# wenzhang-dev/bitcaskDB

Hardware: AMD Instinct MI355X
Metric: WAL record decode+CRC GiB/s (device-resident), 4 KiB values, 1/2/4/8 MI355X (higher is better)
Workload: dtype u8; 1 GPU; config B: 1073743514 B WAL segment per GPU, NsSize 20, 100 B keys, 4 KiB values, device-resident decode+CRC+record parse; seg_bytes=1073743514, records=253846, fragments=286402, parallelism=one independent segment per GPU x1

## Files before the change

### bitcaskdb_amd/csrc/bcw_decode.hip

```cpp
#include <hip/hip_runtime.h>

#include <cstdint>

#include "bcw_internal.h"
#include "bcw_parse.h"

namespace bcw {

enum { M_FIRST_BAD = 0,
       M_NE = 1,
       M_NFRAGS = 4, M_DONE_CRC = 5,
       M_T_CRC0 = 10, M_T_FIN = 11,
       M_ABORT = 12,
       M_BAD_CRC = 14,
       M_BAD_TYPE = 15 };

__device__ __forceinline__ uint32_t rotl32(uint32_t x, int r) { return (x << r) | (x >> (32 - r)); }

__device__ __forceinline__ void read_header(const uint8_t* __restrict__ seg, uint64_t seg_len, uint64_t off,
                                            uint32_t& crc, uint32_t& len, uint32_t& type) {
  const uint64_t a = off & ~3ull;
  uint32_t w0, w1, w2;
  if (a + 12 <= seg_len) {
    const uint32_t* q = reinterpret_cast<const uint32_t*>(seg + a);
    w0 = q[0]; w1 = q[1]; w2 = q[2];
  } else {
    uint32_t b[12];
#pragma unroll
    for (int i = 0; i < 12; ++i) b[i] = (a + i < seg_len) ? seg[a + i] : 0u;
    w0 = b[0] | b[1] << 8 | b[2] << 16 | b[3] << 24;
    w1 = b[4] | b[5] << 8 | b[6] << 16 | b[7] << 24;
    w2 = b[8] | b[9] << 8 | b[10] << 16 | b[11] << 24;
  }
  const uint32_t sh = (uint32_t)(off & 3);
  crc = __builtin_amdgcn_alignbyte(w1, w0, sh);
  const uint32_t t = __builtin_amdgcn_alignbyte(w2, w1, sh);
  len = t & 0xffffu;
  type = (t >> 16) & 0xffu;
}

// ... 408 lines not shown
}
__device__ __forceinline__ uint32_t apply_fwd(const uint32_t* __restrict__ fwd, uint32_t lane, uint32_t x) {
  const uint8_t* b = reinterpret_cast<const uint8_t*>(fwd);
  const uint32_t lane4 = 4u * lane;
  auto at = [&](int i) -> uint32_t {
    const uint32_t sh = 4 * i >= 8 ? (x >> (4 * i - 8)) : (x << (8 - 4 * i));
    return *reinterpret_cast<const uint32_t*>(b + (((sh & 0xf00u) | lane4) + 4096u * (uint32_t)i));
  };
  const uint32_t r0 = at(0), r1 = at(1), r2 = at(2), r3 = at(3), r4 = at(4), r5 = at(5), r6 = at(6), r7 = at(7);
  return xor3(xor3(r0, r1, r2), xor3(r3, r4, r5), r6) ^ r7;
}
__device__ __forceinline__ uint32_t apply_op(const uint32_t* __restrict__ c, uint32_t x) {
  uint32_t r = 0;
#pragma unroll
  for (int i = 0; i < 8; ++i) r ^= c[i * 16 + ((x >> (4 * i)) & 15u)];
  return r;
}

__device__ __forceinline__ uint4 load16_slow(const uint8_t* __restrict__ seg, uint64_t seg_len, int64_t o) {
  uint64_t lo = 0, hi = 0;
#pragma unroll 1
  for (int i = 0; i < 16; ++i) {
    const int64_t q = o + i;
    const uint64_t byte = (q >= 0 && (uint64_t)q < seg_len) ? seg[q] : 0u;
    if (i < 8) lo |= byte << (8 * i); else hi |= byte << (8 * (i - 8));
  }
  return make_uint4((uint32_t)lo, (uint32_t)(lo >> 32), (uint32_t)hi, (uint32_t)(hi >> 32));
}
__device__ __forceinline__ uint4 load16_safe(const uint8_t* __restrict__ seg, uint64_t seg_len, int64_t o) {
  if (o >= 0 && (uint64_t)o + 16 <= seg_len) return *reinterpret_cast<const uint4*>(seg + o);
  return load16_slow(seg, seg_len, o);
}


template <int N>
__device__ __forceinline__ uint32_t reg_byte(const uint32_t (&h)[N], uint32_t pos) {
  uint32_t t[N];
#pragma unroll
  for (int i = 0; i < N; ++i) t[i] = h[i];
  const uint32_t wi = pos >> 2;
  int n = N;
#pragma unroll
  for (int bit = 0; bit < 6; ++bit) {
    if (n <= 1) break;
    const bool hi = (wi >> bit) & 1u;
#pragma unroll
    for (int i = 0; i < (N + 1) / 2; ++i) {
      if (i < (n + 1) / 2) t[i] = (2 * i + 1 < n) ? (hi ? t[2 * i + 1] : t[2 * i]) : t[2 * i];
    }
    n = (n + 1) / 2;
  }
  return (t[0] >> (8u * (pos & 3u))) & 0xffu;
}

constexpr int kHeadWords = 16;
constexpr int kTailWords = 8;

__device__ __attribute__((noinline)) uint32_t walk_byte(const uint8_t* __restrict__ seg, const Frag* __restrict__ frags,
                                                        uint32_t start_off, uint32_t f_first, uint32_t f_last,
                                                        uint64_t pos) {
  uint64_t beg = 0;
  for (uint32_t cf = f_first;; ++cf) {
    const Frag f = frags[cf];
    if (pos < beg + f.len || cf >= f_last)
      return seg[(uint64_t)start_off + (uint64_t)f.blk * kBlock + f.start + (pos - beg)];
    beg += f.len;
  }
}

struct RegReader {
  uint32_t h[kHeadWords];
  uint32_t t[kTailWords];
  uint32_t nhead;
  uint64_t tstart;
  uint64_t tend;
  const uint8_t* seg;
  const Frag* frags;
  uint32_t start_off;
  uint32_t f_first, f_last;
  __device__ __forceinline__ uint32_t operator()(uint64_t pos) {
    if (pos < nhead) return reg_byte(h, (uint32_t)pos);
    if (pos >= tstart && pos < tend) return reg_byte(t, (uint32_t)(pos - tstart));
    return walk_byte(seg, frags, start_off, f_first, f_last, pos);
  }
};

template <int N>
__device__ __forceinline__ void load_words(const uint8_t* __restrict__ seg, uint64_t seg_len, uint64_t base,
                                           uint32_t (&w)[N]) {
  if (base + 4u * N <= seg_len) {
#pragma unroll
    for (int k = 0; k < N / 4; ++k) {
      uint4 v;
      __builtin_memcpy(&v, seg + base + 16 * k, 16);
      w[4 * k + 0] = v.x; w[4 * k + 1] = v.y; w[4 * k + 2] = v.z; w[4 * k + 3] = v.w;
    }
  } else {
#pragma unroll
    for (int k = 0; k < N / 4; ++k) {
      const uint4 v = load16_safe(seg, seg_len, (int64_t)(base + 16 * k));
      w[4 * k + 0] = v.x; w[4 * k + 1] = v.y; w[4 * k + 2] = v.z; w[4 * k + 3] = v.w;
    }
  }
}

struct EmitArgs {
  const uint8_t* seg;
  uint64_t seg_len;
  bcw_decode_params p;
  const Frag* frags;
  const uint32_t* fbase;
  const uint32_t* rbase;
  const uint2* bsum;
  bcw_record_table tab;
  uint64_t* misc;
  uint32_t kb_flags;
  uint64_t* kb_stamps;
};


struct EmitState {
  uint64_t acc;
  int64_t nzb;
  uint32_t nzk, nzs;
  uint64_t rec;
};
__device__ __forceinline__ uint2 emit_prefetch(const EmitArgs& A, uint64_t b0, uint32_t lane) {
  return b0 > lane ? A.bsum[b0 - 1 - lane] : make_uint2(0xffff0000u, kSumHasE);
}

__device__ __forceinline__ EmitState emit_state(const EmitArgs& A, uint64_t b0, uint32_t lane, uint2 s, uint32_t rec) {
  EmitState st{0, -1, 0, 0, rec};
  uint64_t acc = 0;
  for (uint64_t top = b0; top > 0;) {
    if (top != b0) {
      const uint64_t q = top - 1 - lane;
      s = top > lane ? A.bsum[q] : make_uint2(0xffff0000u, kSumHasE);
    }
    const uint64_t he = __ballot((s.y & kSumHasE) != 0u);
    const uint32_t stop = he ? (uint32_t)__builtin_ctzll(he) : 63u;
    const bool contrib = lane <= stop;
    uint32_t ta = contrib ? (s.x & 0xffffu) : 0u;
#pragma unroll
    for (int d = 32; d >= 1; d >>= 1) ta += (uint32_t)__shfl_xor((int)ta, d, 64);
    acc += (uint32_t)__builtin_amdgcn_readfirstlane(ta);
    const uint64_t nzm = __ballot(contrib && (s.x >> 16) != 0xffffu);
    if (nzm) {
      const uint32_t L = 63u - __builtin_clzll(nzm);
      st.nzb = (int64_t)(top - 1 - L);
      st.nzk = (uint32_t)__builtin_amdgcn_readlane((int)(s.x >> 16), L);
      st.nzs = (uint32_t)__builtin_amdgcn_readlane((int)(s.y & 0xffffu), L);
    }
    if (he) break;
    top = top > 64 ? top - 64 : 0;
  }
  st.acc = acc;
  return st;
}

template <bool NOSTORE = false, bool NOPARSE = false, typename Hook>
__device__ __forceinline__ void emit_chunks(const EmitArgs& A, const EmitState& es, uint64_t f0, uint64_t f1,
                                            uint32_t lane, Hook&& hook) {
  if (f0 >= f1) {
    hook();
    return;
  }
  const Frag* __restrict__ frags = A.frags;
  const uint32_t start_off = A.p.start_off;
  uint64_t acc = es.acc, off = 0;
  uint32_t first = 0;
  if (es.nzb >= 0) {
    off = (uint64_t)start_off + (uint64_t)es.nzb * kBlock + es.nzs;
    first = A.fbase[es.nzb] + es.nzk;
  }
  uint64_t rec = es.rec;
  const bool hint = A.p.mode == BCW_MODE_HINT;
  for (uint64_t c0 = f0; c0 < f1; c0 += 64) {
    const uint64_t g = c0 + lane;
    const bool valid = g < f1;
    const uint4 fr = reinterpret_cast<const uint4*>(frags)[valid ? g : f1 - 1];
    if (c0 == f0) hook();
    Frag f;
    __builtin_memcpy(&f, &fr, sizeof f);
    if (!valid) f = Frag{};
    const uint32_t len = valid ? f.len : 0u;
    const uint64_t D = (uint64_t)start_off + (uint64_t)f.blk * kBlock + f.start;
    const bool isE = valid && (f.type == BCW_RECORD_FULL || f.type == BCW_RECORD_LAST);
    const uint64_t E = __ballot(isE);
    const uint64_t NZ = __ballot(valid && len > 0);
    const uint32_t S = wave_add_scan(len, lane);
    const uint64_t below = (lane == 0) ? 0ull : (~0ull >> (64 - lane));
    const uint64_t pm = E & below;
    const int prev = pm ? 63 - __builtin_clzll(pm) : -1;
    const uint32_t S_prev = __shfl(S, prev < 0 ? 0 : prev, 64);
    const uint64_t between = (uint64_t)(S - len) - (prev < 0 ? 0u : S_prev);
    const uint64_t acc_before = (prev < 0 ? acc : 0ull) + between;
    const uint64_t range = prev < 0 ? below : (below & ~(~0ull >> (63 - prev)));
    const uint64_t nzr = NZ & range;
    const int fnz = nzr ? __builtin_ctzll(nzr) : 0;
    const uint64_t D_fnz = __shfl(D, fnz, 64);
    const uint64_t V = __ballot(valid);
    const int last_valid = V ? 63 - __builtin_clzll(V) : -1;
    const uint32_t S_tot = __shfl(S, last_valid < 0 ? 0 : last_valid, 64);
// ... 17 lines not shown
      }
    }
    uint64_t foff;
    uint32_t ffrag;
    if (acc_before == 0) { foff = D; ffrag = (uint32_t)g; }
    else if (prev < 0 && acc > 0) { foff = off; ffrag = first; }
    else { foff = D_fnz; ffrag = (uint32_t)(c0 + fnz); }
    const bool full = f.type == BCW_RECORD_FULL;
    const uint32_t src = full ? (uint32_t)g : ffrag;
    const bool src_here = src >= c0 && src < c0 + 64;
    const uint32_t sw0 = (uint32_t)__shfl((int)f.blk, src_here ? (int)(src - c0) : (int)lane, 64);
    const uint32_t sw1 = (uint32_t)__shfl((int)((uint32_t)f.start | ((uint32_t)f.len << 16)),
                                          src_here ? (int)(src - c0) : (int)lane, 64);
    const bool nx_here = src + 1u >= c0 && src + 1u < c0 + 64;
    const uint32_t sx0 = (uint32_t)__shfl((int)f.blk, nx_here ? (int)(src + 1u - c0) : (int)lane, 64);
    const uint32_t sx1 = (uint32_t)__shfl((int)((uint32_t)f.start | ((uint32_t)f.len << 16)),
                                          nx_here ? (int)(src + 1u - c0) : (int)lane, 64);
    if (isE) {
      const uint64_t size = full ? (uint64_t)len : acc_before + len;
      const uint64_t r = rec + __builtin_popcountll(E & below);
      Frag fs = f;
      if (!full) {
        if (src_here) { fs.blk = sw0; fs.start = (uint16_t)sw1; fs.len = (uint16_t)(sw1 >> 16); }
        else fs = frags[src];
      }
      RegReader rd;
      const uint64_t a0 = (uint64_t)start_off + (uint64_t)fs.blk * kBlock + fs.start;
      uint64_t want = size < 64u ? size : 64u;
      if (want > fs.len) want = fs.len;
      rd.nhead = (uint32_t)want;
      load_words(A.seg, A.seg_len, a0, rd.h);
      rd.tstart = rd.tend = ~0ull;
      if (hint) {
        uint64_t nt = size < 32u ? size : 32u;
        if (nt > len) nt = len;
        rd.tstart = size - nt;
        load_words(A.seg, A.seg_len, D + len - nt, rd.t);
      } else if (want < (size < 64u ? size : 64u)) {
        Frag f2;
        if (nx_here) { f2.blk = sx0; f2.start = (uint16_t)sx1; f2.len = (uint16_t)(sx1 >> 16); }
        else f2 = frags[src + 1u];
        load_words(A.seg, A.seg_len, (uint64_t)start_off + (uint64_t)f2.blk * kBlock + f2.start, rd.t);
        uint64_t n2 = f2.len < 32u ? f2.len : 32u;
        if (n2 > size - want) n2 = size - want;
        rd.tstart = want;
        rd.tend = want + n2;
      } else {
#pragma unroll
        for (int k = 0; k < kTailWords; ++k) rd.t[k] = 0;
      }
      rd.seg = A.seg; rd.frags = frags; rd.start_off = start_off;
      rd.f_first = src; rd.f_last = (uint32_t)g;
      uint8_t status, hdr, flags, etag_off;
      uint64_t key_len, val_len, meta_len, expire, aux0, aux1;
      if (NOPARSE) {
        status = 0; hdr = (uint8_t)rd.h[0]; flags = (uint8_t)rd.h[5]; etag_off = 0;
        key_len = rd.h[6] ^ rd.h[9]; val_len = rd.h[7] ^ rd.h[12]; meta_len = rd.h[8] ^ rd.h[15]; expire = rd.h[10];
        aux0 = rd.t[0]; aux1 = rd.t[1];
      } else {
        parse_record(A.p, rd, size, status, hdr, flags, etag_off, key_len, val_len, meta_len, expire, aux0, aux1);
      }
      const bcw_record_table& tab = A.tab;
      if (NOSTORE) {
        if (status == 0xeeu) tab.foff[r] = foff ^ size ^ expire ^ aux0 ^ aux1 ^ key_len ^ val_len ^ meta_len ^ hdr ^ flags ^ etag_off;
      } else if (r < tab.capacity) {
        tab.foff[r] = foff;
        tab.size[r] = size;
        tab.expire[r] = expire;
        if (tab.aux0) tab.aux0[r] = aux0;
        if (tab.aux1) tab.aux1[r] = aux1;
        tab.key_len[r] = (uint32_t)key_len;
        tab.val_len[r] = (uint32_t)val_len;
        tab.meta_len[r] = (uint32_t)meta_len;
        tab.first_frag[r] = src;
        tab.emit_frag[r] = (uint32_t)g;
        tab.hdr_size[r] = hdr;
        tab.flags[r] = flags;
        tab.etag_off[r] = etag_off;
        tab.status[r] = status;
      }
      if (status != BCW_ST_OK) atomicMin((unsigned long long*)&A.misc[M_FIRST_BAD], (unsigned long long)r);
    }
    rec += __builtin_popcountll(E);
    acc = acc2;
    off = off2;
    first = first2;
  }
}

struct ItemMeta {
  uint64_t bb;
  uint2 s;
  uint32_t f0, f1, rec;
};
__device__ __forceinline__ uint32_t ld_const(const uint32_t* p, uint64_t i) {
  return ((const __attribute__((address_space(4))) uint32_t*)p)[i];
}
__device__ __forceinline__ ItemMeta item_meta(const EmitArgs& A, uint64_t it, uint64_t bpw, uint64_t cb0, uint64_t cb1,
                                              uint32_t lane) {
  ItemMeta m;
  m.bb = cb0 + it * bpw < cb1 ? cb0 + it * bpw : cb1 - 1;
  const uint64_t be = m.bb + bpw < cb1 ? m.bb + bpw : cb1;
  m.s = emit_prefetch(A, m.bb, lane);
  m.f0 = ld_const(A.fbase, m.bb);
  m.f1 = ld_const(A.fbase, be);
  m.rec = ld_const(A.rbase, m.bb);
  return m;
}

__device__ __forceinline__ void finalize(const EmitArgs& A, uint64_t nblocks, uint64_t frag_cap, uint32_t tail_panic, uint64_t gen,
                         bcw_decode_result* __restrict__ res, uint32_t lane) {
  uint64_t* misc = A.misc;
  const uint64_t bad_crc = __hip_atomic_load(&misc[M_BAD_CRC], __ATOMIC_RELAXED, __HIP_MEMORY_SCOPE_AGENT);
  const uint64_t bad_type = __hip_atomic_load(&misc[M_BAD_TYPE], __ATOMIC_RELAXED, __HIP_MEMORY_SCOPE_AGENT);
  const uint64_t fb = __hip_atomic_load(&misc[M_FIRST_BAD], __ATOMIC_RELAXED, __HIP_MEMORY_SCOPE_AGENT);
  const uint64_t nfr = __hip_atomic_load(&misc[M_NFRAGS], __ATOMIC_RELAXED, __HIP_MEMORY_SCOPE_AGENT);
  const uint64_t abort_site = __hip_atomic_load(&misc[M_ABORT], __ATOMIC_RELAXED, __HIP_MEMORY_SCOPE_AGENT);
  const uint64_t err = bad_crc < bad_type ? bad_crc : bad_type;
  uint64_t lim = err < frag_cap ? err : frag_cap;
  uint64_t nrec = __hip_atomic_load(&misc[M_NE], __ATOMIC_RELAXED, __HIP_MEMORY_SCOPE_AGENT);
  if (lim < nfr && abort_site == 0ull) {
    uint64_t lo = 0, hi = nblocks;
    while (hi - lo > 1) {
      const uint64_t step = (hi - lo + 63) / 64;
      const uint64_t q = lo + (uint64_t)lane * step;
      const bool le = q < hi && A.fbase[q] <= lim;
      const uint64_t m = __ballot(le);
      const uint32_t L = m ? 63u - __builtin_clzll(m) : 0u;
      lo = lo + (uint64_t)L * step;
      hi = lo + step < hi ? lo + step : hi;
    }
    uint64_t cnt = 0;
    for (uint64_t c0 = A.fbase[lo]; c0 < lim; c0 += 64) {
      const uint64_t g = c0 + lane;
      const uint32_t ty = g < lim ? A.frags[g].type : 0u;
      cnt += (uint64_t)__builtin_popcountll(__ballot(ty == BCW_RECORD_FULL || ty == BCW_RECORD_LAST));
    }
    nrec = (uint64_t)A.rbase[lo] + cnt;
  }
  if (lane != 0) return;
  bcw_decode_result r{};
  r.n_records = nrec;
  r.n_records_total = nrec;
  r.err_frag = err;
  r.err_class = err == ~0ull ? BCW_ERR_NONE : (bad_crc <= bad_type ? BCW_ERR_CRC : BCW_ERR_TYPE);
  r.n_frags = err != ~0ull ? err + 1 : nfr;
  if (r.err_class == BCW_ERR_NONE && tail_panic) r.err_class = BCW_ERR_PANIC;
  if (abort_site != 0ull) {
    r.err_class = BCW_ERR_INTERNAL;
    r.err_frag = abort_site;
    r.n_records = r.n_records_total = 0;
    nrec = 0;
  }
  r.err_file_off = 0;
  if (err != ~0ull && err < frag_cap && abort_site == 0ull) {
    const Frag f = A.frags[err];
    r.err_file_off = (uint64_t)A.p.start_off + (uint64_t)f.blk * kBlock + f.start - kHdr;
  }
  r.first_bad_record = fb < nrec ? (int32_t)(fb < 0x7fffffffull ? fb : 0x7fffffffull) : -1;
  r.n_blocks = nblocks;
  r.retry_frag_capacity = (nfr > frag_cap && abort_site == 0ull) ? nfr : 0;
  r.generation = gen;
  *res = r;
  if (abort_site != 0ull) misc[M_NFRAGS] = 0;
  misc[M_DONE_CRC] = 0;
  misc[M_BAD_CRC] = ~0ull;
  misc[M_FIRST_BAD] = ~0ull;
  misc[M_BAD_TYPE] = ~0ull;
  misc[M_ABORT] = 0;
}

struct StreamFrag {
  int64_t gs, ge;
  uint32_t J;
};

struct SliceLane2 {
  uint32_t base;
  uint32_t sel[4];
};
__device__ __forceinline__ SliceLane2 slice_lane2(uint32_t lane) {
  SliceLane2 s;
  const uint32_t g = (lane >> 3) & 3u, copy = lane & 7u;
  s.base = 0;
#pragma unroll
  for (uint32_t k = 0; k < 4; ++k) {
    const uint32_t slot = (k + g) & 3u;
    s.base |= (slot * 32u + copy * 4u) << (8u * k);
    s.sel[k] = 0x0c0c0000u | ((4u + slot) << 8) | k;
  }
  return s;
}
// ... 240 lines not shown
      const float d = fminf(fmaxf(rintf((wy - 65536.0f) / 256.0f), -51.0f), 64.0f);
      xb->w[y] = (uint32_t)(65536 + 256 * (int32_t)d);
    }
    xb->t[y] = 0;
    xb->n[y] = 0;
  }
}

template <int ABL = 0>
__global__ __launch_bounds__(kCrcThreads) void k_crc(const uint8_t* __restrict__ seg, uint64_t seg_len,
                                                     uint32_t start_off, uint64_t nblocks,
                                                     const uint32_t* __restrict__ fbase, uint8_t* __restrict__ fok,
                                                     const uint4* __restrict__ srec,
                                                     uint64_t frag_cap, Tables tabs, EmitArgs ea,
                                                     uint32_t tail_panic, uint64_t gen,
                                                     bcw_decode_result* __restrict__ res,
                                                     uint64_t* __restrict__ misc, uint64_t cb0, uint64_t cb1,
                                                     uint32_t nwg_total, const uint32_t* __restrict__ wstart,
                                                     XBal* __restrict__ xb) {
  __shared__ __attribute__((aligned(16))) uint32_t lds[kS2Image];
  __shared__ CrcTail s_tail;
  __shared__ uint32_t s_wdone;
  __shared__ uint32_t s_eq;
  __shared__ __attribute__((aligned(16))) uint32_t s_rem[kCrcWaves];
  __shared__ uint32_t s_sdone;
  __shared__ unsigned long long s_tsum;
  __shared__ uint64_t s_t0;
  const uint32_t tid = threadIdx.x;
  const uint32_t lane = tid & 63u;
  const uint32_t wave = __builtin_amdgcn_readfirstlane(tid >> 6);
  if (tid < (uint32_t)kCrcWaves) s_rem[tid] = 0;
  if (ea.kb_stamps && lane == 0) {
    uint64_t* q = ea.kb_stamps + 8 * ((uint64_t)blockIdx.x * kCrcWaves + wave);
    q[4] = wall_clock64();
    q[5] = __builtin_amdgcn_s_memtime();
    q[7] = ((uint64_t)__builtin_amdgcn_s_getreg(20 | (31 << 11)) << 32) | __builtin_amdgcn_s_getreg(4 | (31 << 11));
  }
  if (tid == 0) {
    s_wdone = 0;
    s_eq = 0;
    s_sdone = 0;
    s_tsum = 0;
    s_t0 = wall_clock64();
    s_tail = CrcTail{ea, res, misc, nblocks, frag_cap, gen, cb0, cb1, tail_panic, nwg_total};
  }
  {
// ... 21 lines not shown
    for (int k2 = 0; k2 < kPer; ++k2) {
      const uint32_t i = tid + k2 * kCrcThreads;
      if (i < kN4) dst4[at(i)] = v[k2];
    }
#pragma unroll
    for (int k2 = 0; k2 < 2; ++k2) {
      const uint32_t t = tid + k2 * kCrcThreads;
      uint4* d = reinterpret_cast<uint4*>(lds + kS2SliceOff + (t >> 3) * 64u + (t & 7u) * 8u);
      d[0] = make_uint4(sv[k2], sv[k2], sv[k2], sv[k2]);
      d[1] = make_uint4(sv[k2], sv[k2], sv[k2], sv[k2]);
    }
  }
  __syncthreads();
  const uint64_t gw = (uint64_t)blockIdx.x * kCrcWaves + wave;
  const uint64_t f0 = wstart[gw];
  uint64_t f1 = wstart[gw + 1];
  if (f1 > frag_cap) f1 = frag_cap;
  if (f0 > f1) f1 = f0;
  const bool aborted = __builtin_amdgcn_readfirstlane(
                           (uint32_t)__hip_atomic_load(&misc[M_ABORT], __ATOMIC_RELAXED, __HIP_MEMORY_SCOPE_AGENT)) != 0u;
  if (aborted) f1 = f0;
  if (blockIdx.x == 0 && tid == 0) misc[M_T_CRC0] = wall_clock64();
  const uint32_t nfr = f1 > f0 ? (uint32_t)(f1 - f0) : 0u;
  uint64_t n_items = 0;
  auto emit_items = [&](uint64_t max_items) {
    asm volatile("" ::: "memory");
    CrcTail T;
    {
      static_assert(sizeof(CrcTail) % 4 == 0, "CrcTail words");
      const uint32_t* src = reinterpret_cast<const uint32_t*>(&s_tail);
      uint32_t* dst = reinterpret_cast<uint32_t*>(&T);
#pragma unroll
      for (int k = 0; k < (int)(sizeof(CrcTail) / 4); ++k) dst[k] = __builtin_amdgcn_readfirstlane(src[k]);
    }
    const EmitArgs& A = T.ea;
    if ((ABL & 8) || (A.kb_flags & 1u) ||
        __builtin_amdgcn_readfirstlane(
            (uint32_t)__hip_atomic_load(&T.misc[M_ABORT], __ATOMIC_RELAXED, __HIP_MEMORY_SCOPE_AGENT)) != 0u)
      return;
    const uint64_t cb0t = T.cb0, cb1t = T.cb1, fcap = T.frag_cap;
    const uint32_t cnt = (uint32_t)(cb1t - cb0t), G = gridDim.x, wg = blockIdx.x;
    const uint64_t fc0 = A.fbase[cb0t], fc1 = A.fbase[cb1t];
    const uint32_t nf_all = (uint32_t)(fc1 > fc0 ? (fc1 - fc0 < fcap ? fc1 - fc0 : fcap) : 0);
    uint32_t bpw = nf_all ? (64u * cnt) / nf_all : cnt;
    if (bpw < 1u) bpw = 1u;
    bpw = __builtin_amdgcn_readfirstlane(bpw);
    const uint32_t cq = cnt / G, cr = cnt % G;
    const uint32_t B0 = cq * wg + (cr * wg) / G, B1 = cq * (wg + 1u) + (cr * (wg + 1u)) / G;
    const uint64_t i0 = __builtin_amdgcn_readfirstlane((B0 + bpw - 1u) / bpw),
                   nitems = __builtin_amdgcn_readfirstlane((B1 + bpw - 1u) / bpw);
    auto deq = [&]() -> uint64_t {
      uint32_t j = 0;
      if (lane == 0) j = atomicAdd(&s_eq, 1u);
      j = __builtin_amdgcn_readfirstlane(j);
      return i0 + j;
    };
    uint64_t taken = 0;
    uint64_t it = deq();
    ItemMeta m = item_meta(A, it, bpw, cb0t, cb1t, lane);
    while (it < nitems) {
      ++taken;
      const EmitState es = emit_state(A, m.bb, lane, m.s, m.rec);
      const uint64_t mf1 = m.f1 < fcap ? m.f1 : fcap;
      uint64_t nx = ~0ull;
      ItemMeta mn = m;
      emit_chunks<(ABL & 4096) != 0, (ABL & 131072) != 0>(A, es, m.f0, mf1, lane, [&]() {
        if (taken < max_items) {
          nx = deq();
          mn = item_meta(A, nx, bpw, cb0t, cb1t, lane);
        }
      });
      it = nx;
      m = mn;
    }
    n_items += taken;
  };
  if (ABL & 64) emit_items(~0ull);
  if (ABL & 16384) {
    for (uint32_t q = 0; q < 4u; ++q) {
      const uint32_t a = nfr * q / 4u, b = nfr * (q + 1u) / 4u;
      stream_verify<(ABL & 8388608) != 0>(seg, seg_len, fok, srec, f0 + a, b - a, lds, lane, misc, s_rem,
                                          (wave & 3u) * 4u + (wave >> 2),
                                          reinterpret_cast<const uint8_t*>(tabs.lds_image2));
    }
  } else if (!(ABL & 32768))
    stream_verify<(ABL & 8388608) != 0>(seg, seg_len, fok, srec, f0, nfr, lds, lane, misc, s_rem,
                                        (wave & 3u) * 4u + (wave >> 2),
                                        reinterpret_cast<const uint8_t*>(tabs.lds_image2));
  __builtin_amdgcn_s_setprio(0);
  if (lane == 0) {
    atomicAdd(&s_tsum, (unsigned long long)(wall_clock64() - s_t0));
    if (atomicAdd(&s_sdone, 1u) == kCrcWaves - 1u) {
      const uint32_t c = blockIdx.x & 7u;
      __hip_atomic_fetch_add(&xb->t[c], (uint64_t)s_tsum, __ATOMIC_RELAXED, __HIP_MEMORY_SCOPE_AGENT);
      __hip_atomic_fetch_add(&xb->n[c], (uint64_t)kCrcWaves, __ATOMIC_RELAXED, __HIP_MEMORY_SCOPE_AGENT);
    }
  }
  if (ea.kb_stamps && lane == 0) {
    uint64_t* q = ea.kb_stamps + 8 * ((uint64_t)blockIdx.x * kCrcWaves + wave);
    q[0] = wall_clock64();
    q[3] = nfr;
  }
  if (!(ABL & 64)) emit_items(~0ull);
  asm volatile("" ::: "memory");
  CrcTail T;
  {
    const uint32_t* src = reinterpret_cast<const uint32_t*>(&s_tail);
    uint32_t* dst = reinterpret_cast<uint32_t*>(&T);
#pragma unroll
    for (int k = 0; k < (int)(sizeof(CrcTail) / 4); ++k) dst[k] = __builtin_amdgcn_readfirstlane(src[k]);
  }
  const EmitArgs& A = T.ea;
  if (A.kb_stamps && lane == 0) {
    uint64_t* q = A.kb_stamps + 8 * ((uint64_t)__builtin_amdgcn_workgroup_id_x() * kCrcWaves + wave);
    q[1] = wall_clock64(); q[2] = n_items;
    q[6] = __builtin_amdgcn_s_memtime();
  }
  asm volatile("s_waitcnt vmcnt(0)" ::: "memory");
  __builtin_amdgcn_fence(__ATOMIC_RELEASE, "workgroup");
  uint32_t order = 0;
  if (lane == 0) order = atomicAdd(&s_wdone, 1u);
  order = __builtin_amdgcn_readlane(order, 0);
  if (order != kCrcWaves - 1) return;
  __builtin_amdgcn_fence(__ATOMIC_ACQUIRE, "workgroup");
  uint64_t gorder = 0;
  if (lane == 0)
    gorder = __hip_atomic_fetch_add(&T.misc[M_DONE_CRC], 1ull, __ATOMIC_RELAXED, __HIP_MEMORY_SCOPE_AGENT);
  gorder = (uint64_t)__shfl((long long)gorder, 0, 64);
  if (gorder != T.nwg_total - 1u) return;
  if (lane == 0) T.misc[M_T_FIN] = wall_clock64();
  const XBalIn xin = xbal_load(xb, lane);
  finalize(A, T.nblocks, T.frag_cap, T.tail_panic, T.gen, T.res, lane);
  xbal_update(xb, lane, xin);
}

__global__ void k_export_frags(const Frag* __restrict__ frags, const uint8_t* __restrict__ fok,
                               const uint64_t* __restrict__ misc, uint64_t cap,
                               uint32_t start_off, bcw_frag_table out, const uint32_t* __restrict__ initc) {
  const uint64_t g = blockIdx.x * (uint64_t)blockDim.x + threadIdx.x;
  const uint64_t n = misc[M_NFRAGS];
  if (g >= n || g >= cap || g >= out.capacity) return;
  const Frag f = frags[g];
  out.data_off[g] = (uint64_t)start_off + (uint64_t)f.blk * kBlock + f.start;
  out.len[g] = f.len;
  const uint32_t u = ~(f.chk ^ initc[f.len]);
  out.stored_crc[g] = ((u >> 15) | (u << 17)) + 0xa282ead8u;
  out.type[g] = f.type;
  out.crc_ok[g] = fok[g];
}



hipError_t launch_decode(const uint8_t* d_seg, const bcw_decode_params& p, const bcw_record_table& t,
// ... 39 lines not shown
```

### bitcaskdb_amd/csrc/bcw_parse.h

```cpp
#pragma once
#include <hip/hip_runtime.h>

#include <cstdint>

#include "bcw.h"

namespace bcw {

template <typename RD>
__device__ __forceinline__ uint64_t uvarint(RD& rd, uint64_t pos, uint64_t len, uint32_t& used) {
  uint64_t x = 0;
  uint32_t s = 0;
#pragma unroll 1
  for (uint32_t i = 0; pos + i < len; ++i) {
    if (i == 10) { used = 0; return 0; }
    const uint32_t b = rd(pos + i);
    if (b < 0x80u) {
      if (i == 9 && b > 1u) { used = 0; return 0; }
      used = i + 1;
      return x | ((uint64_t)b << s);
    }
    x |= (uint64_t)(b & 0x7fu) << s;
    s += 7;
  }
  used = 0;
  return 0;
}

template <typename RD>
__device__ __forceinline__ void parse_record(const bcw_decode_params& p, RD& rd, uint64_t len, uint8_t& status,
                                             uint8_t& hdr, uint8_t& flags, uint8_t& etag_off, uint64_t& key_len,
                                             uint64_t& val_len, uint64_t& meta_len, uint64_t& expire, uint64_t& aux0,
                                             uint64_t& aux1) {
  uint32_t used;
  status = BCW_ST_OK;
  hdr = flags = etag_off = 0;
  key_len = val_len = meta_len = expire = aux0 = aux1 = 0;
  if (p.mode == BCW_MODE_RECORD) {
    const uint64_t min_hdr = 1ull + p.ns_size + 1ull + 3ull;
    if (len < min_hdr) { status = BCW_ST_INVALID; return; }
    const uint64_t header = rd(0);
    uint64_t o = 1 + p.ns_size;
    const uint32_t flag = rd(o);
    ++o;
    key_len = uvarint(rd, o, len, used); o += used;
    val_len = uvarint(rd, o, len, used); o += used;
    meta_len = uvarint(rd, o, len, used); o += used;
    const uint64_t etag_len = (flag & 1u) ? 0 : p.etag_size;
    uint64_t expire_size = 0;
    hdr = (uint8_t)header; flags = (uint8_t)flag; etag_off = (uint8_t)o;
    if ((flag & 2u) == 0) {
      if (o + etag_len > len) { status = BCW_ST_PANIC; return; }
      expire = uvarint(rd, o + etag_len, len, used);
// ... 6 lines not shown
    const uint64_t s1 = key_len + val_len;
    const uint64_t s2 = s1 + meta_len;
    const bool wrapped = (s1 < key_len) || (s2 < s1);
    if ((int64_t)key_len < 0 || (int64_t)val_len < 0 || (int64_t)meta_len < 0 || wrapped) status = BCW_ST_PANIC;
    else if (key_len > 0xffffffffull || val_len > 0xffffffffull || meta_len > 0xffffffffull || len > 0xffffffffull)
      status = BCW_ST_UNSUPPORTED;
  } else {
    if (len < (uint64_t)p.ns_size + 5ull) { status = BCW_ST_INVALID; return; }
    int64_t o = p.ns_size;
    key_len = uvarint(rd, (uint64_t)o, len, used);
    o += used;
    const int64_t key_off = o;
    o = (int64_t)((uint64_t)o + key_len);
    hdr = (uint8_t)key_off;
    if (o < 0 || o > (int64_t)len) { status = BCW_ST_PANIC; return; }
    expire = uvarint(rd, (uint64_t)o, len, used); o += used;
    aux0 = uvarint(rd, (uint64_t)o, len, used); o += used;
    aux1 = uvarint(rd, (uint64_t)o, len, used); o += used;
    if (o != (int64_t)len) status = BCW_ST_INVALID;
    else if ((int64_t)key_len < 0) status = BCW_ST_PANIC;
  }
}

}
```

Baseline: 4978 GiB/s.

## Add branch-free windowed record parser fast path with explicit global address-space loads

Adds a fast path that parses the record header from a small preloaded byte window, decoding the uvarints with bit tricks instead of a byte-by-byte reader loop. The old register-reader parse remains only as a wave-level fallback and reloads its arguments from LDS to reduce register pressure. Loads and stores are also marked with the global or constant address space, and some indices are narrowed to 32 bits, so the compiler can emit global_load/s_load instead of flat accesses. The risk is subtle mismatches against the reference parser on edge cases, such as long varints or records that span fragments, and extra code size.

```diff
diff --git a/bitcaskdb_amd/csrc/bcw_decode.hip b/bitcaskdb_amd/csrc/bcw_decode.hip
--- a/bitcaskdb_amd/csrc/bcw_decode.hip
+++ b/bitcaskdb_amd/csrc/bcw_decode.hip
@@ -16,6 +16,41 @@
        M_BAD_TYPE = 15 };
 
 __device__ __forceinline__ uint32_t rotl32(uint32_t x, int r) { return (x << r) | (x >> (32 - r)); }
+
+#define BCW_GLOBAL __attribute__((address_space(1)))
+template <typename T>
+__device__ __forceinline__ BCW_GLOBAL T* gp(T* p) { return (BCW_GLOBAL T*)p; }
+typedef uint32_t v4u __attribute__((ext_vector_type(4)));
+typedef uint32_t v2u __attribute__((ext_vector_type(2)));
+typedef v4u v4u_unaligned __attribute__((aligned(1)));
+typedef uint64_t u64_unaligned __attribute__((aligned(1)));
+__device__ __forceinline__ uint4 ldg16(const void* p) {
+  const v4u v = *(const BCW_GLOBAL v4u*)p;
+  return make_uint4(v.x, v.y, v.z, v.w);
+}
+__device__ __forceinline__ uint4 ldg16_u(const void* p) {
+  const v4u v = *(const BCW_GLOBAL v4u_unaligned*)p;
+  return make_uint4(v.x, v.y, v.z, v.w);
+}
+__device__ __forceinline__ uint64_t ldg8_u(const void* p) { return *(const BCW_GLOBAL u64_unaligned*)p; }
+__device__ __forceinline__ uint2 ldg8(const uint2* p) {
+  const v2u v = *(const BCW_GLOBAL v2u*)p;
+  return make_uint2(v.x, v.y);
+}
+template <typename T>
+__device__ __forceinline__ T lds_copy(const T* p) {
+  static_assert(sizeof(T) % 4 == 0, "whole words");
+  const __attribute__((address_space(3))) uint32_t* s = (const __attribute__((address_space(3))) uint32_t*)p;
+  uint32_t w[sizeof(T) / 4];
+#pragma unroll
+  for (int k = 0; k < (int)(sizeof(T) / 4); ++k) w[k] = s[k];
+  T out;
+  __builtin_memcpy(&out, w, sizeof(T));
+  return out;
+}
+__device__ __forceinline__ uint64_t ldg_relaxed(const uint64_t* p) {
+  return __hip_atomic_load(gp(p), __ATOMIC_RELAXED, __HIP_MEMORY_SCOPE_AGENT);
+}
 
 __device__ __forceinline__ void read_header(const uint8_t* __restrict__ seg, uint64_t seg_len, uint64_t off,
                                             uint32_t& crc, uint32_t& len, uint32_t& type) {
@@ -470,13 +505,13 @@
 #pragma unroll 1
   for (int i = 0; i < 16; ++i) {
     const int64_t q = o + i;
-    const uint64_t byte = (q >= 0 && (uint64_t)q < seg_len) ? seg[q] : 0u;
+    const uint64_t byte = (q >= 0 && (uint64_t)q < seg_len) ? gp(seg)[q] : 0u;
     if (i < 8) lo |= byte << (8 * i); else hi |= byte << (8 * (i - 8));
   }
   return make_uint4((uint32_t)lo, (uint32_t)(lo >> 32), (uint32_t)hi, (uint32_t)(hi >> 32));
 }
 __device__ __forceinline__ uint4 load16_safe(const uint8_t* __restrict__ seg, uint64_t seg_len, int64_t o) {
-  if (o >= 0 && (uint64_t)o + 16 <= seg_len) return *reinterpret_cast<const uint4*>(seg + o);
+  if (o >= 0 && (uint64_t)o + 16 <= seg_len) return ldg16(seg + o);
   return load16_slow(seg, seg_len, o);
 }
 
@@ -504,18 +539,25 @@
 constexpr int kHeadWords = 16;
 constexpr int kTailWords = 8;
 
+__device__ __forceinline__ Frag load_frag(const Frag* frags, uint64_t i);
 __device__ __attribute__((noinline)) uint32_t walk_byte(const uint8_t* __restrict__ seg, const Frag* __restrict__ frags,
                                                         uint32_t start_off, uint32_t f_first, uint32_t f_last,
                                                         uint64_t pos) {
   uint64_t beg = 0;
   for (uint32_t cf = f_first;; ++cf) {
-    const Frag f = frags[cf];
+    const Frag f = load_frag(frags, cf);
     if (pos < beg + f.len || cf >= f_last)
-      return seg[(uint64_t)start_off + (uint64_t)f.blk * kBlock + f.start + (pos - beg)];
+      return gp(seg)[(uint64_t)start_off + (uint64_t)f.blk * kBlock + f.start + (pos - beg)];
     beg += f.len;
   }
 }
 
+__device__ __forceinline__ Frag load_frag(const Frag* frags, uint64_t i) {
+  const uint4 v = ldg16(frags + i);
+  Frag f;
+  __builtin_memcpy(&f, &v, sizeof f);
+  return f;
+}
 struct RegReader {
   uint32_t h[kHeadWords];
   uint32_t t[kTailWords];
@@ -539,8 +581,7 @@
   if (base + 4u * N <= seg_len) {
 #pragma unroll
     for (int k = 0; k < N / 4; ++k) {
-      uint4 v;
-      __builtin_memcpy(&v, seg + base + 16 * k, 16);
+      const uint4 v = ldg16_u(seg + base + 16 * k);
       w[4 * k + 0] = v.x; w[4 * k + 1] = v.y; w[4 * k + 2] = v.z; w[4 * k + 3] = v.w;
     }
   } else {
@@ -550,6 +591,10 @@
       w[4 * k + 0] = v.x; w[4 * k + 1] = v.y; w[4 * k + 2] = v.z; w[4 * k + 3] = v.w;
     }
   }
+}
+
+__device__ __forceinline__ uint32_t ld_const(const uint32_t* p, uint64_t i) {
+  return ((const __attribute__((address_space(4))) uint32_t*)p)[i];
 }
 
 struct EmitArgs {
@@ -574,7 +619,7 @@
   uint64_t rec;
 };
 __device__ __forceinline__ uint2 emit_prefetch(const EmitArgs& A, uint64_t b0, uint32_t lane) {
-  return b0 > lane ? A.bsum[b0 - 1 - lane] : make_uint2(0xffff0000u, kSumHasE);
+  return b0 > lane ? ldg8(A.bsum + (b0 - 1 - lane)) : make_uint2(0xffff0000u, kSumHasE);
 }
 
 __device__ __forceinline__ EmitState emit_state(const EmitArgs& A, uint64_t b0, uint32_t lane, uint2 s, uint32_t rec) {
@@ -583,7 +628,7 @@
   for (uint64_t top = b0; top > 0;) {
     if (top != b0) {
       const uint64_t q = top - 1 - lane;
-      s = top > lane ? A.bsum[q] : make_uint2(0xffff0000u, kSumHasE);
+      s = top > lane ? ldg8(A.bsum + q) : make_uint2(0xffff0000u, kSumHasE);
     }
     const uint64_t he = __ballot((s.y & kSumHasE) != 0u);
     const uint32_t stop = he ? (uint32_t)__builtin_ctzll(he) : 63u;
@@ -607,8 +652,8 @@
 }
 
 template <bool NOSTORE = false, bool NOPARSE = false, typename Hook>
-__device__ __forceinline__ void emit_chunks(const EmitArgs& A, const EmitState& es, uint64_t f0, uint64_t f1,
-                                            uint32_t lane, Hook&& hook) {
+__device__ __forceinline__ void emit_chunks(const EmitArgs& A, const EmitArgs* lds_args, const EmitState& es,
+                                            uint64_t f0, uint64_t f1, uint32_t lane, Hook&& hook) {
   if (f0 >= f1) {
     hook();
     return;
@@ -619,14 +664,14 @@
   uint32_t first = 0;
   if (es.nzb >= 0) {
     off = (uint64_t)start_off + (uint64_t)es.nzb * kBlock + es.nzs;
-    first = A.fbase[es.nzb] + es.nzk;
+    first = ld_const(A.fbase, (uint64_t)es.nzb) + es.nzk;
   }
   uint64_t rec = es.rec;
   const bool hint = A.p.mode == BCW_MODE_HINT;
   for (uint64_t c0 = f0; c0 < f1; c0 += 64) {
     const uint64_t g = c0 + lane;
     const bool valid = g < f1;
-    const uint4 fr = reinterpret_cast<const uint4*>(frags)[valid ? g : f1 - 1];
+    const uint4 fr = ldg16(frags + (valid ? g : f1 - 1));
     if (c0 == f0) hook();
     Frag f;
     __builtin_memcpy(&f, &fr, sizeof f);
@@ -690,64 +735,96 @@
       Frag fs = f;
       if (!full) {
         if (src_here) { fs.blk = sw0; fs.start = (uint16_t)sw1; fs.len = (uint16_t)(sw1 >> 16); }
-        else fs = frags[src];
+        else fs = load_frag(frags, src);
       }
-      RegReader rd;
       const uint64_t a0 = (uint64_t)start_off + (uint64_t)fs.blk * kBlock + fs.start;
-      uint64_t want = size < 64u ? size : 64u;
-      if (want > fs.len) want = fs.len;
-      rd.nhead = (uint32_t)want;
-      load_words(A.seg, A.seg_len, a0, rd.h);
-      rd.tstart = rd.tend = ~0ull;
-      if (hint) {
-        uint64_t nt = size < 32u ? size : 32u;
-        if (nt > len) nt = len;
-        rd.tstart = size - nt;
-        load_words(A.seg, A.seg_len, D + len - nt, rd.t);
-      } else if (want < (size < 64u ? size : 64u)) {
-        Frag f2;
-        if (nx_here) { f2.blk = sx0; f2.start = (uint16_t)sx1; f2.len = (uint16_t)(sx1 >> 16); }
-        else f2 = frags[src + 1u];
-        load_words(A.seg, A.seg_len, (uint64_t)start_off + (uint64_t)f2.blk * kBlock + f2.start, rd.t);
-        uint64_t n2 = f2.len < 32u ? f2.len : 32u;
-        if (n2 > size - want) n2 = size - want;
-        rd.tstart = want;
-        rd.tend = want + n2;
-      } else {
-#pragma unroll
-        for (int k = 0; k < kTailWords; ++k) rd.t[k] = 0;
+      const uint64_t avail = size < fs.len ? size : (uint64_t)fs.len;
+      uint8_t status = BCW_ST_OK, hdr = 0, flags = 0, etag_off = 0;
+      uint64_t key_len = 0, val_len = 0, meta_len = 0, expire = 0, aux0 = 0, aux1 = 0;
+      bool fast = false;
+      bcw_decode_params pw = A.p;
+      pw.base_time = 0;
+      if (!NOPARSE && !hint) {
+        uint32_t flag_pos = 1u + A.p.ns_size;
+        asm("" : "+v"(flag_pos));
+        const uint64_t wb = a0 + flag_pos, web = wb + A.p.etag_size;
+        if (web + kRecWindow <= A.seg_len) {
+          const uint32_t header = gp(A.seg)[a0];
+          const uint4 w01 = ldg16_u(A.seg + wb);
+          uint64_t w[3] = {w01.x | (uint64_t)w01.y << 32, w01.z | (uint64_t)w01.w << 32, ldg8_u(A.seg + wb + 16)};
+          uint64_t we[3] = {0, 0, 0};
+          if (A.p.etag_size != 0u) {
+            const uint4 e01 = ldg16_u(A.seg + web);
+            we[0] = e01.x | (uint64_t)e01.y << 32;
+            we[1] = e01.z | (uint64_t)e01.w << 32;
+            we[2] = ldg8_u(A.seg + web + 16);
+          }
+          fast = parse_record_window(pw, flag_pos, header, w, we, size, avail, status, hdr, flags, etag_off, key_len,
+                                     val_len, meta_len, expire);
+        }
       }
-      rd.seg = A.seg; rd.frags = frags; rd.start_off = start_off;
-      rd.f_first = src; rd.f_last = (uint32_t)g;
-      uint8_t status, hdr, flags, etag_off;
-      uint64_t key_len, val_len, meta_len, expire, aux0, aux1;
-      if (NOPARSE) {
-        status = 0; hdr = (uint8_t)rd.h[0]; flags = (uint8_t)rd.h[5]; etag_off = 0;
-        key_len = rd.h[6] ^ rd.h[9]; val_len = rd.h[7] ^ rd.h[12]; meta_len = rd.h[8] ^ rd.h[15]; expire = rd.h[10];
-        aux0 = rd.t[0]; aux1 = rd.t[1];
-      } else {
-        parse_record(A.p, rd, size, status, hdr, flags, etag_off, key_len, val_len, meta_len, expire, aux0, aux1);
+      if (__ballot(!fast) != 0ull) {
+        if (!fast) {
+          asm volatile("" ::: "memory");
+          const EmitArgs G = lds_copy(lds_args);
+          RegReader rd;
+          const uint64_t want = avail < 64u ? avail : 64u;
+          rd.nhead = (uint32_t)want;
+          load_words(G.seg, G.seg_len, (uint64_t)G.p.start_off + (uint64_t)fs.blk * kBlock + fs.start, rd.h);
+          rd.tstart = rd.tend = ~0ull;
+          if (hint) {
+            uint64_t nt = size < 32u ? size : 32u;
+            if (nt > len) nt = len;
+            rd.tstart = size - nt;
+            load_words(G.seg, G.seg_len, (uint64_t)G.p.start_off + (uint64_t)f.blk * kBlock + f.start + len - nt, rd.t);
+          } else if (want < (size < 64u ? size : 64u)) {
+            Frag f2;
+            if (nx_here) { f2.blk = sx0; f2.start = (uint16_t)sx1; f2.len = (uint16_t)(sx1 >> 16); }
+            else f2 = load_frag(G.frags, src + 1u);
+            load_words(G.seg, G.seg_len, (uint64_t)G.p.start_off + (uint64_t)f2.blk * kBlock + f2.start, rd.t);
+            uint64_t n2 = f2.len < 32u ? f2.len : 32u;
+            if (n2 > size - want) n2 = size - want;
+            rd.tstart = want;
+            rd.tend = want + n2;
+          } else {
+#pragma unroll
+            for (int k = 0; k < kTailWords; ++k) rd.t[k] = 0;
+          }
+          rd.seg = G.seg; rd.frags = G.frags; rd.start_off = G.p.start_off;
+          rd.f_first = src; rd.f_last = (uint32_t)g;
+          if (NOPARSE) {
+            status = 0; hdr = (uint8_t)rd.h[0]; flags = (uint8_t)rd.h[5]; etag_off = 0;
+            key_len = rd.h[6] ^ rd.h[9]; val_len = rd.h[7] ^ rd.h[12]; meta_len = rd.h[8] ^ rd.h[15]; expire = rd.h[10];
+            aux0 = rd.t[0]; aux1 = rd.t[1];
+          } else {
+            parse_record(G.p, rd, size, status, hdr, flags, etag_off, key_len, val_len, meta_len, expire, aux0, aux1);
+          }
+        }
       }
-      const bcw_record_table& tab = A.tab;
+      asm volatile("" ::: "memory");
+      const bcw_record_table tab = lds_copy(&lds_args->tab);
+      if (fast && (flags & 2u) == 0) expire += lds_copy(&lds_args->p.base_time);
       if (NOSTORE) {
-        if (status == 0xeeu) tab.foff[r] = foff ^ size ^ expire ^ aux0 ^ aux1 ^ key_len ^ val_len ^ meta_len ^ hdr ^ flags ^ etag_off;
+        if (status == 0xeeu)
+          gp(tab.foff)[r] = foff ^ size ^ expire ^ aux0 ^ aux1 ^ key_len ^ val_len ^ meta_len ^ hdr ^ flags ^ etag_off;
       } else if (r < tab.capacity) {
-        tab.foff[r] = foff;
-        tab.size[r] = size;
-        tab.expire[r] = expire;
-        if (tab.aux0) tab.aux0[r] = aux0;
-        if (tab.aux1) tab.aux1[r] = aux1;
-        tab.key_len[r] = (uint32_t)key_len;
-        tab.val_len[r] = (uint32_t)val_len;
-        tab.meta_len[r] = (uint32_t)meta_len;
-        tab.first_frag[r] = src;
-        tab.emit_frag[r] = (uint32_t)g;
-        tab.hdr_size[r] = hdr;
-        tab.flags[r] = flags;
-        tab.etag_off[r] = etag_off;
-        tab.status[r] = status;
+        gp(tab.foff)[r] = foff;
+        gp(tab.size)[r] = size;
+        gp(tab.expire)[r] = expire;
+        if (tab.aux0) gp(tab.aux0)[r] = aux0;
+        if (tab.aux1) gp(tab.aux1)[r] = aux1;
+        gp(tab.key_len)[r] = (uint32_t)key_len;
+        gp(tab.val_len)[r] = (uint32_t)val_len;
+        gp(tab.meta_len)[r] = (uint32_t)meta_len;
+        gp(tab.first_frag)[r] = src;
+        gp(tab.emit_frag)[r] = (uint32_t)g;
+        gp(tab.hdr_size)[r] = hdr;
+        gp(tab.flags)[r] = flags;
+        gp(tab.etag_off)[r] = etag_off;
+        gp(tab.status)[r] = status;
       }
-      if (status != BCW_ST_OK) atomicMin((unsigned long long*)&A.misc[M_FIRST_BAD], (unsigned long long)r);
+      if (status != BCW_ST_OK)
+        __hip_atomic_fetch_min(gp(&A.misc[M_FIRST_BAD]), (uint64_t)r, __ATOMIC_RELAXED, __HIP_MEMORY_SCOPE_AGENT);
     }
     rec += __builtin_popcountll(E);
     acc = acc2;
@@ -761,9 +838,6 @@
   uint2 s;
   uint32_t f0, f1, rec;
 };
-__device__ __forceinline__ uint32_t ld_const(const uint32_t* p, uint64_t i) {
-  return ((const __attribute__((address_space(4))) uint32_t*)p)[i];
-}
 __device__ __forceinline__ ItemMeta item_meta(const EmitArgs& A, uint64_t it, uint64_t bpw, uint64_t cb0, uint64_t cb1,
                                               uint32_t lane) {
   ItemMeta m;
@@ -779,32 +853,32 @@
 __device__ __forceinline__ void finalize(const EmitArgs& A, uint64_t nblocks, uint64_t frag_cap, uint32_t tail_panic, uint64_t gen,
                          bcw_decode_result* __restrict__ res, uint32_t lane) {
   uint64_t* misc = A.misc;
-  const uint64_t bad_crc = __hip_atomic_load(&misc[M_BAD_CRC], __ATOMIC_RELAXED, __HIP_MEMORY_SCOPE_AGENT);
-  const uint64_t bad_type = __hip_atomic_load(&misc[M_BAD_TYPE], __ATOMIC_RELAXED, __HIP_MEMORY_SCOPE_AGENT);
-  const uint64_t fb = __hip_atomic_load(&misc[M_FIRST_BAD], __ATOMIC_RELAXED, __HIP_MEMORY_SCOPE_AGENT);
-  const uint64_t nfr = __hip_atomic_load(&misc[M_NFRAGS], __ATOMIC_RELAXED, __HIP_MEMORY_SCOPE_AGENT);
-  const uint64_t abort_site = __hip_atomic_load(&misc[M_ABORT], __ATOMIC_RELAXED, __HIP_MEMORY_SCOPE_AGENT);
+  const uint64_t bad_crc = ldg_relaxed(&misc[M_BAD_CRC]);
+  const uint64_t bad_type = ldg_relaxed(&misc[M_BAD_TYPE]);
+  const uint64_t fb = ldg_relaxed(&misc[M_FIRST_BAD]);
+  const uint64_t nfr = ldg_relaxed(&misc[M_NFRAGS]);
+  const uint64_t abort_site = ldg_relaxed(&misc[M_ABORT]);
   const uint64_t err = bad_crc < bad_type ? bad_crc : bad_type;
   uint64_t lim = err < frag_cap ? err : frag_cap;
-  uint64_t nrec = __hip_atomic_load(&misc[M_NE], __ATOMIC_RELAXED, __HIP_MEMORY_SCOPE_AGENT);
+  uint64_t nrec = ldg_relaxed(&misc[M_NE]);
   if (lim < nfr && abort_site == 0ull) {
     uint64_t lo = 0, hi = nblocks;
     while (hi - lo > 1) {
       const uint64_t step = (hi - lo + 63) / 64;
       const uint64_t q = lo + (uint64_t)lane * step;
-      const bool le = q < hi && A.fbase[q] <= lim;
+      const bool le = q < hi && gp(A.fbase)[q] <= lim;
       const uint64_t m = __ballot(le);
       const uint32_t L = m ? 63u - __builtin_clzll(m) : 0u;
       lo = lo + (uint64_t)L * step;
       hi = lo + step < hi ? lo + step : hi;
     }
     uint64_t cnt = 0;
-    for (uint64_t c0 = A.fbase[lo]; c0 < lim; c0 += 64) {
+    for (uint64_t c0 = ld_const(A.fbase, lo); c0 < lim; c0 += 64) {
       const uint64_t g = c0 + lane;
-      const uint32_t ty = g < lim ? A.frags[g].type : 0u;
+      const uint32_t ty = g < lim ? load_frag(A.frags, g).type : 0u;
       cnt += (uint64_t)__builtin_popcountll(__ballot(ty == BCW_RECORD_FULL || ty == BCW_RECORD_LAST));
     }
-    nrec = (uint64_t)A.rbase[lo] + cnt;
+    nrec = (uint64_t)ld_const(A.rbase, lo) + cnt;
   }
   if (lane != 0) return;
   bcw_decode_result r{};
@@ -822,20 +896,26 @@
   }
   r.err_file_off = 0;
   if (err != ~0ull && err < frag_cap && abort_site == 0ull) {
-    const Frag f = A.frags[err];
+    const Frag f = load_frag(A.frags, err);
     r.err_file_off = (uint64_t)A.p.start_off + (uint64_t)f.blk * kBlock + f.start - kHdr;
   }
   r.first_bad_record = fb < nrec ? (int32_t)(fb < 0x7fffffffull ? fb : 0x7fffffffull) : -1;
   r.n_blocks = nblocks;
   r.retry_frag_capacity = (nfr > frag_cap && abort_site == 0ull) ? nfr : 0;
   r.generation = gen;
-  *res = r;
-  if (abort_site != 0ull) misc[M_NFRAGS] = 0;
-  misc[M_DONE_CRC] = 0;
-  misc[M_BAD_CRC] = ~0ull;
-  misc[M_FIRST_BAD] = ~0ull;
-  misc[M_BAD_TYPE] = ~0ull;
-  misc[M_ABORT] = 0;
+  {
+    static_assert(sizeof(bcw_decode_result) % 8 == 0, "bcw_decode_result words");
+    uint64_t rw[sizeof(bcw_decode_result) / 8];
+    __builtin_memcpy(rw, &r, sizeof r);
+#pragma unroll
+    for (int k = 0; k < (int)(sizeof r / 8); ++k) gp(reinterpret_cast<uint64_t*>(res))[k] = rw[k];
+  }
+  if (abort_site != 0ull) gp(misc)[M_NFRAGS] = 0;
+  gp(misc)[M_DONE_CRC] = 0;
+  gp(misc)[M_BAD_CRC] = ~0ull;
+  gp(misc)[M_FIRST_BAD] = ~0ull;
+  gp(misc)[M_BAD_TYPE] = ~0ull;
+  gp(misc)[M_ABORT] = 0;
 }
 
 struct StreamFrag {
@@ -1122,6 +1202,7 @@
   __shared__ CrcTail s_tail;
   __shared__ uint32_t s_wdone;
   __shared__ uint32_t s_eq;
+  __shared__ uint32_t s_bc[kCrcWaves];
   __shared__ __attribute__((aligned(16))) uint32_t s_rem[kCrcWaves];
   __shared__ uint32_t s_sdone;
   __shared__ unsigned long long s_tsum;
@@ -1189,8 +1270,15 @@
   if (aborted) f1 = f0;
   if (blockIdx.x == 0 && tid == 0) misc[M_T_CRC0] = wall_clock64();
   const uint32_t nfr = f1 > f0 ? (uint32_t)(f1 - f0) : 0u;
+  auto lane0_bcast = [&](uint32_t v) -> uint32_t {
+    typedef volatile __attribute__((address_space(3))) uint32_t* lds_word;
+    lds_word w = (lds_word)&s_bc[wave];
+    if (lane == 0) *w = v;
+    __builtin_amdgcn_wave_barrier();
+    return __builtin_amdgcn_readfirstlane(*w);
+  };
   uint64_t n_items = 0;
-  auto emit_items = [&](uint64_t max_items) {
+  auto emit_items = [&](uint32_t max_items) {
     asm volatile("" ::: "memory");
     CrcTail T;
     {
@@ -1201,37 +1289,35 @@
       for (int k = 0; k < (int)(sizeof(CrcTail) / 4); ++k) dst[k] = __builtin_amdgcn_readfirstlane(src[k]);
     }
     const EmitArgs& A = T.ea;
-    if ((ABL & 8) || (A.kb_flags & 1u) ||
-        __builtin_amdgcn_readfirstlane(
-            (uint32_t)__hip_atomic_load(&T.misc[M_ABORT], __ATOMIC_RELAXED, __HIP_MEMORY_SCOPE_AGENT)) != 0u)
-      return;
+    if ((ABL & 8) || (A.kb_flags & 1u)) return;
+    const uint64_t abort_site = ldg_relaxed(&T.misc[M_ABORT]);
     const uint64_t cb0t = T.cb0, cb1t = T.cb1, fcap = T.frag_cap;
     const uint32_t cnt = (uint32_t)(cb1t - cb0t), G = gridDim.x, wg = blockIdx.x;
-    const uint64_t fc0 = A.fbase[cb0t], fc1 = A.fbase[cb1t];
+    const uint64_t fc0 = ld_const(A.fbase, cb0t), fc1 = ld_const(A.fbase, cb1t);
     const uint32_t nf_all = (uint32_t)(fc1 > fc0 ? (fc1 - fc0 < fcap ? fc1 - fc0 : fcap) : 0);
     uint32_t bpw = nf_all ? (64u * cnt) / nf_all : cnt;
     if (bpw < 1u) bpw = 1u;
     bpw = __builtin_amdgcn_readfirstlane(bpw);
     const uint32_t cq = cnt / G, cr = cnt % G;
     const uint32_t B0 = cq * wg + (cr * wg) / G, B1 = cq * (wg + 1u) + (cr * (wg + 1u)) / G;
-    const uint64_t i0 = __builtin_amdgcn_readfirstlane((B0 + bpw - 1u) / bpw),
+    const uint32_t i0 = __builtin_amdgcn_readfirstlane((B0 + bpw - 1u) / bpw),
                    nitems = __builtin_amdgcn_readfirstlane((B1 + bpw - 1u) / bpw);
-    auto deq = [&]() -> uint64_t {
+    auto deq = [&]() -> uint32_t {
       uint32_t j = 0;
       if (lane == 0) j = atomicAdd(&s_eq, 1u);
-      j = __builtin_amdgcn_readfirstlane(j);
-      return i0 + j;
+      return i0 + lane0_bcast(j);
     };
-    uint64_t taken = 0;
-    uint64_t it = deq();
+    uint32_t taken = 0;
+    uint32_t it = deq();
     ItemMeta m = item_meta(A, it, bpw, cb0t, cb1t, lane);
+    if (__builtin_amdgcn_readfirstlane((uint32_t)abort_site) != 0u) return;
     while (it < nitems) {
       ++taken;
       const EmitState es = emit_state(A, m.bb, lane, m.s, m.rec);
       const uint64_t mf1 = m.f1 < fcap ? m.f1 : fcap;
-      uint64_t nx = ~0ull;
+      uint32_t nx = ~0u;
       ItemMeta mn = m;
-      emit_chunks<(ABL & 4096) != 0, (ABL & 131072) != 0>(A, es, m.f0, mf1, lane, [&]() {
+      emit_chunks<(ABL & 4096) != 0, (ABL & 131072) != 0>(A, &s_tail.ea, es, m.f0, mf1, lane, [&]() {
         if (taken < max_items) {
           nx = deq();
           mn = item_meta(A, nx, bpw, cb0t, cb1t, lane);
@@ -1242,7 +1328,7 @@
     }
     n_items += taken;
   };
-  if (ABL & 64) emit_items(~0ull);
+  if (ABL & 64) emit_items(~0u);
   if (ABL & 16384) {
     for (uint32_t q = 0; q < 4u; ++q) {
       const uint32_t a = nfr * q / 4u, b = nfr * (q + 1u) / 4u;
@@ -1268,7 +1354,7 @@
     q[0] = wall_clock64();
     q[3] = nfr;
   }
-  if (!(ABL & 64)) emit_items(~0ull);
+  if (!(ABL & 64)) emit_items(~0u);
   asm volatile("" ::: "memory");
   CrcTail T;
   {
@@ -1279,7 +1365,7 @@
   }
   const EmitArgs& A = T.ea;
   if (A.kb_stamps && lane == 0) {
-    uint64_t* q = A.kb_stamps + 8 * ((uint64_t)__builtin_amdgcn_workgroup_id_x() * kCrcWaves + wave);
+    BCW_GLOBAL uint64_t* q = gp(A.kb_stamps) + 8 * ((uint64_t)__builtin_amdgcn_workgroup_id_x() * kCrcWaves + wave);
     q[1] = wall_clock64(); q[2] = n_items;
     q[6] = __builtin_amdgcn_s_memtime();
   }
@@ -1287,15 +1373,16 @@
   __builtin_amdgcn_fence(__ATOMIC_RELEASE, "workgroup");
   uint32_t order = 0;
   if (lane == 0) order = atomicAdd(&s_wdone, 1u);
-  order = __builtin_amdgcn_readlane(order, 0);
+  order = lane0_bcast(order);
   if (order != kCrcWaves - 1) return;
   __builtin_amdgcn_fence(__ATOMIC_ACQUIRE, "workgroup");
-  uint64_t gorder = 0;
+  uint32_t gorder = 0;
   if (lane == 0)
-    gorder = __hip_atomic_fetch_add(&T.misc[M_DONE_CRC], 1ull, __ATOMIC_RELAXED, __HIP_MEMORY_SCOPE_AGENT);
-  gorder = (uint64_t)__shfl((long long)gorder, 0, 64);
+    gorder = (uint32_t)__hip_atomic_fetch_add(gp(&T.misc[M_DONE_CRC]), 1ull, __ATOMIC_RELAXED,
+                                              __HIP_MEMORY_SCOPE_AGENT);
+  gorder = lane0_bcast(gorder);
   if (gorder != T.nwg_total - 1u) return;
-  if (lane == 0) T.misc[M_T_FIN] = wall_clock64();
+  if (lane == 0) gp(T.misc)[M_T_FIN] = wall_clock64();
   const XBalIn xin = xbal_load(xb, lane);
   finalize(A, T.nblocks, T.frag_cap, T.tail_panic, T.gen, T.res, lane);
   xbal_update(xb, lane, xin);
diff --git a/bitcaskdb_amd/csrc/bcw_parse.h b/bitcaskdb_amd/csrc/bcw_parse.h
--- a/bitcaskdb_amd/csrc/bcw_parse.h
+++ b/bitcaskdb_amd/csrc/bcw_parse.h
@@ -8,7 +8,7 @@
 namespace bcw {
 
 template <typename RD>
-__device__ __forceinline__ uint64_t uvarint(RD& rd, uint64_t pos, uint64_t len, uint32_t& used) {
+__host__ __device__ __forceinline__ uint64_t uvarint(RD& rd, uint64_t pos, uint64_t len, uint32_t& used) {
   uint64_t x = 0;
   uint32_t s = 0;
 #pragma unroll 1
@@ -28,7 +28,7 @@
 }
 
 template <typename RD>
-__device__ __forceinline__ void parse_record(const bcw_decode_params& p, RD& rd, uint64_t len, uint8_t& status,
+__host__ __device__ __forceinline__ void parse_record(const bcw_decode_params& p, RD& rd, uint64_t len, uint8_t& status,
                                              uint8_t& hdr, uint8_t& flags, uint8_t& etag_off, uint64_t& key_len,
                                              uint64_t& val_len, uint64_t& meta_len, uint64_t& expire, uint64_t& aux0,
                                              uint64_t& aux1) {
@@ -81,4 +81,71 @@
   }
 }
 
+
+__host__ __device__ __forceinline__ bool uvarint_w32(uint32_t w, uint32_t& val, uint32_t& used) {
+  const uint32_t t = ~w & 0x80808080u;
+  uint32_t v = w & (t ^ (t - 1u)) & 0x7f7f7f7fu;
+  v = ((v & 0x7f007f00u) >> 1) | (v & 0x007f007fu);
+  v = ((v & 0x3fff0000u) >> 2) | (v & 0x00003fffu);
+  val = v;
+  used = ((uint32_t)__builtin_ctz(t | 0x80000000u) >> 3) + 1u;
+  return t != 0u;
 }
+__host__ __device__ __forceinline__ bool uvarint_w64(uint64_t w, uint64_t& val, uint32_t& used) {
+  const uint64_t t = ~w & 0x8080808080808080ull;
+  uint64_t v = w & (t ^ (t - 1ull)) & 0x7f7f7f7f7f7f7f7full;
+  v = ((v & 0x7f007f007f007f00ull) >> 1) | (v & 0x007f007f007f007full);
+  v = ((v & 0x3fff00003fff0000ull) >> 2) | (v & 0x00003fff00003fffull);
+  v = ((v & 0x0fffffff00000000ull) >> 4) | (v & 0x000000000fffffffull);
+  val = v;
+  used = ((uint32_t)__builtin_ctzll(t | (1ull << 63)) >> 3) + 1u;
+  return t != 0ull;
+}
+__host__ __device__ __forceinline__ void window_skip(uint64_t (&w)[3], uint32_t n) {
+  const uint32_t s = 8u * n;
+  w[0] = (w[0] >> s) | (w[1] << (64u - s));
+  w[1] = (w[1] >> s) | (w[2] << (64u - s));
+  w[2] >>= s;
+}
+
+constexpr uint32_t kRecWindow = 24;
+
+__host__ __device__ __forceinline__ bool parse_record_window(const bcw_decode_params& p, uint32_t flag_pos,
+                                                             uint32_t header, const uint64_t (&w_in)[3],
+                                                             const uint64_t (&we_in)[3],
+                                                             uint64_t len, uint64_t avail, uint8_t& status,
+                                                             uint8_t& hdr, uint8_t& flags, uint8_t& etag_off,
+                                                             uint64_t& key_len, uint64_t& val_len, uint64_t& meta_len,
+                                                             uint64_t& expire) {
+  uint64_t w[3] = {w_in[0], w_in[1], w_in[2]};
+  uint64_t we[3] = {we_in[0], we_in[1], we_in[2]};
+  const bool has_etag = p.etag_size != 0u;
+  const uint32_t flag = (uint32_t)w[0] & 0xffu;
+  uint32_t kl, vl, ml, n1, n2, n3;
+  bool ok = uvarint_w32((uint32_t)(w[0] >> 8), kl, n1);
+  window_skip(w, 1u + n1);
+  if (has_etag) window_skip(we, 1u + n1);
+  ok &= uvarint_w32((uint32_t)w[0], vl, n2);
+  window_skip(w, n2);
+  if (has_etag) window_skip(we, n2);
+  ok &= uvarint_w32((uint32_t)w[0], ml, n3);
+  window_skip(w, n3);
+  if (has_etag) window_skip(we, n3);
+  const uint32_t o = flag_pos + 1u + n1 + n2 + n3;
+  const uint32_t etag_len = (flag & 1u) ? 0u : p.etag_size;
+  uint64_t ex = 0;
+  uint32_t ne = 0;
+  if ((flag & 2u) == 0) {
+    ok &= uvarint_w64(has_etag && etag_len ? we[0] : w[0], ex, ne);
+    ex += p.base_time;
+  }
+  const uint64_t cur_hdr = (uint64_t)o + etag_len + ne;
+  if (!ok || cur_hdr > avail) return false;
+  hdr = (uint8_t)header; flags = (uint8_t)flag; etag_off = (uint8_t)o;
+  key_len = kl; val_len = vl; meta_len = ml; expire = ex;
+  if (cur_hdr != (uint64_t)header || cur_hdr + ((uint64_t)kl + vl + ml) != len) status = BCW_ST_INVALID;
+  else status = len > 0xffffffffull ? BCW_ST_UNSUPPORTED : BCW_ST_OK;
+  return true;
+}
+
+}
```

After: 5026 GiB/s (median of 6 runs). About the same (+1.0%).
